# jizongFox/Self-paced-Contrastive-Learning

Measured on AMD Instinct MI355X. Metric: pretrain slices/sec/node (UNet+InfoNCE, 224^2, bs=32/GPU), higher is better.
Workload: dtype bf16; 1 GPU; BASELINE.json configs[1]: self-paced pretrain step, UNet base (max_channel=256) encoder to Conv5 + ProjectionHead(256,256,256) + SelfPacedSupConLoss(soft, partition labels, correct_grad) fwd+bwd + RAdam; slices_per_gpu=32, images_per_gpu_step=64, image=1x224x224, global_batch=32, parallelism=dp1, params=1311056, hipgraph=epocher, capture_steps=3

## Files before the change

### include/spcl_hip.h

```cpp
#ifndef SPCL_HIP_H
#define SPCL_HIP_H
#include <stddef.h>
#include <stdint.h>
#ifdef __cplusplus
extern "C" {
#endif

#define SPCL_F32 0
#define SPCL_BF16 1

#define SPCL_OK 0
#define SPCL_EINVAL (-1)
#define SPCL_ELAUNCH (-2)
#define SPCL_EUNSUPPORTED (-3)

#define SPCL_ABI_VERSION 37
int spcl_abi_version(void);
const char* spcl_last_error(void);

size_t spcl_supcon_workspace_bytes(int n, int d);
int spcl_supcon_forward(const float* z1, const float* z2, const float* labels, const float* mask, int n, int d,
                        float temperature, int sp_mode, float gamma, int correct_grad, float* ws, float* out,
                        void* stream);
int spcl_supcon_backward(const float* labels, const float* mask, int n, int d, float temperature, int sp_mode,
                         float gamma, const float* ws_fwd, float* ws_bwd, const float* out_fwd,
                         const float* grad_out, float* dz1, float* dz2, void* stream);
size_t spcl_supcon_bwd_workspace_bytes(int n, int d);
int spcl_supcon_unit_gradient_block(int n, int d, size_t* offset_floats, int* row_pitch);
int spcl_supcon_forward_heads(int K, const float* z1, const float* z2, size_t z_stride, const float* labels, int n,
                              int d, float temperature, int sp_mode, const float* gammas, int correct_grad, float* ws,
                              size_t ws_stride, float* out, void* stream);
int spcl_supcon_rows_supported(int n, int d);
int spcl_supcon_forward_rows(int K, const float* o1, const float* o2, size_t o_stride, const float* labels, int n, int d,
                             float temperature, int sp_mode, const float* gammas, int correct_grad, float* ws,
                             size_t ws_stride, float* out, void* stream);
int spcl_supcon_backward_heads(int K, const float* labels, int n, int d, float temperature, int sp_mode,
                               const float* gammas, const float* ws_fwd, size_t ws_stride, float* ws_bwd,
                               size_t wsb_stride, const float* out_fwd, const float* grad_out, float* dz1, float* dz2,
                               size_t z_stride, void* stream);
int spcl_supcon_materialize(const float* labels, const float* mask, int n, int d, float temperature, int sp_mode,
                            float gamma, const float* ws_fwd, float* sim_logits, float* sim_exp, float* pos_mask,
                            float* neg_mask, float* sp_mask, void* stream);

size_t spcl_supcon_xpos_workspace_bytes(int n, int d);
int spcl_supcon_xpos_forward(const float* z1, const float* z2, const float* labels, const float* mask, int n, int d,
                             float temperature, float* ws, float* out, void* stream);
int spcl_supcon_xpos_backward(const float* z1, const float* z2, int n, int d, float temperature, const float* ws,
                              const float* grad_out, float* dz1, float* dz2, void* stream);

// ... 188 lines not shown
int spcl_conv3x3_dgrad_bnstats(const void* dy, int dtype, int N, int H, int W, int CinK, int CoutS, const void* w_packed,
                               void* g, const void* y2, const float* scale2, const float* shift2, const float* mean2,
                               float* rows2, void* stream);

int spcl_image_autocorr_rows(int N, int H, int W);
int spcl_image_autocorr(const float* image, int N, int H, int W, float* out, void* stream);
int spcl_conv_dgrad_bnstats_image_supported(int dtype, int N, int H, int W, int CinK, int CoutS);
int spcl_conv3x3_dgrad_bnstats_image(const void* dy, int dtype, int N, int H, int W, int CinK, int CoutS,
                                     const void* w_packed, void* g, const void* y2, const float* scale2,
                                     const float* shift2, const float* mean2, const float* image, float* rows11,
                                     void* stream);
int spcl_conv16_bwd_fused_supported(int dtype, int N, int H, int W, int CinK, int CoutS);
int spcl_conv16_bwd_fused_splits(int N, int H, int W);
int spcl_conv16_bwd_fused(const void* dy, int dtype, int N, int H, int W, const void* w_packed_dgrad, const void* y2,
                          const float* scale2, const float* shift2, const float* mean2, const float* image,
                          float* rows11, float* partial, float* dw_oihw, int Cin, int Cout, float* wg_rows,
                          const float* acorr, int nacorr, float* acorr16, void* stream);
int spcl_conv16_bwd_fused_image_supported(int dtype, int N, int H, int W, int CinK, int CoutS);
int spcl_conv16_bwd_fused_image(const void* dy, int dtype, int N, int H, int W, const void* w_packed_dgrad,
                                const void* w_packed_image, const float* scale2, const float* shift2, const float* mean2,
                                const float* image, float* rows11, float* partial, float* dw_oihw, int Cin, int Cout,
                                float* wg_rows, const float* acorr, int nacorr, float* acorr16, void* stream);
int spcl_conv16_bwd_fused_image_pooled_supported(int dtype, int N, int H, int W, int CinK, int CoutS, int training);
int spcl_conv16_bwd_fused_image_pooled(const void* y, const void* dpool, const float* rows, int nrows, int dtype, int N, int H,
                                       int W, const float* st4, int training, long long* acc, float* dgamma, float* dbeta,
                                       const void* w_packed_dgrad, const void* w_packed_image, const float* scale2,
                                       const float* shift2, const float* mean2, const float* image, float* rows11,
                                       float* partial, float* dw_oihw, int Cin, int Cout, float* wg_rows, const float* acorr,
                                       int nacorr, float* acorr16, void* stream);
int spcl_bnrelu_backward_wgrows_image3(const float* wg_rows, int nwg, const float* acorr, int nacorr, const float* w_oihw,
                                       int N, int H, int W, int C, int CS, const float* mean, const float* invstd,
                                       const float* scale, int training, float* ws, float* dgamma, float* dbeta,
                                       float* dw, void* stream);
size_t spcl_bnrelu_image3_workspace_bytes(int CS);
int spcl_bnrelu_backward_rows_image3(const float* rows11, int nrows, const float* acorr, int nacorr, const float* w_oihw,
                                     int N, int H, int W, int C, int CS, const float* mean, const float* invstd,
                                     const float* scale, int training, float* ws, float* dgamma, float* dbeta, float* dw,
                                     void* stream);

int spcl_conv_dgrad_poolstats_supported(int dtype, int N, int H, int W, int CinK, int CoutS, int H2, int W2);
int spcl_conv3x3_dgrad_poolstats(const void* dy, int dtype, int N, int H, int W, int CinK, int CoutS, const void* w_packed,
                                 void* g, const void* y2, int H2, int W2, const float* scale2, const float* shift2,
                                 const float* mean2, float* rows2, void* stream);
int spcl_bnrelu_pool_backward_rows(const void* y, const void* dpool, const float* rows, int nrows, int dtype, int N, int H,
                                   int W, int C, int CS, const float* mean, const float* invstd, const float* scale,
                                   const float* shift, int training, float* ws, float* dgamma, float* dbeta, void* dy,
                                   void* stream);
int spcl_bnrelu_backward_rows(const void* y, const void* dact, const float* image, const float* rows, int nrows, int dtype,
                              int N, int H, int W, int C, int CS, const float* mean, const float* invstd,
                              const float* scale, const float* shift, int training, float* ws, float* dgamma,
                              float* dbeta, void* dy, float* dw, void* stream);


int spcl_conv1x1_forward(const void* x, int dtype, size_t npix, int C, int CS, int K, const float* w, const float* b,
                         float* out, void* stream);
size_t spcl_conv1x1_bwd_workspace_bytes(int C, int K);
int spcl_conv1x1_backward(const void* x, const float* dout, int dtype, size_t npix, int C, int CS, int K, const float* w,
                          void* dx, float* dw, float* db, float* ws, void* stream);
int spcl_conv1x1_forward_bn(const void* y, int dtype, size_t npix, int C, int CS, int K, const float* scale,
                            const float* shift, const float* w, const float* b, float* out, void* stream);
int spcl_conv1x1_bwd_rows(size_t npix);
int spcl_conv1x1_backward_bn(const void* y, const float* dout, int dtype, size_t npix, int C, int CS, int K,
                             const float* scale, const float* shift, const float* mean, const float* w, void* dact,
                             float* dw, float* db, float* ws, float* rows, void* stream);
int spcl_softmax_forward(const float* logits, size_t npix, int K, float* prob, void* stream);
int spcl_softmax_backward(const float* prob, const float* dprob, size_t npix, int K, float* dlogits, void* stream);
// ... 320 lines not shown
```

### self-paced-contrastive-learning_amd/functional.py

```python
from __future__ import annotations

import collections
import ctypes
import math
import os
import struct
from ctypes import c_double, c_float, c_int

import torch

from . import native as _n

SP_NONE, SP_HARD, SP_SOFT = 0, 1, 2


def take_grad_sink(param, needed: bool = True):
    if not needed or param is None:
        return None
    sink = getattr(param, "_grad_sink", None)
    if sink is None or not getattr(param, "_grad_sink_armed", False):
        return None
    if sink.shape != param.shape or sink.dtype != torch.float32 or not sink.is_contiguous() or sink.device != param.device:
        return None
    param._grad_sink_armed = False
# ... 1150 lines not shown

class DeferredWgrads:

    def __init__(self):
        self.items, self.keep, self.targets = [], [], set()
        self.tails = []

    def add(self, x_store, dy, scale, shift, sink, N, H, W, cin, cin_s, cout, cout_s, in_mode, x2=None, x_up2=False):
        it = _n.WgradItem(x_store.data_ptr(), dy.data_ptr(), scale.data_ptr() if scale is not None else None,
                          shift.data_ptr() if shift is not None else None, sink.data_ptr(), N, H, W, cin, cin_s, cout,
                          cout_s, in_mode, x2.data_ptr() if x2 is not None else None, 1 if x_up2 else 0)
        self.items.append(it)
        self.keep.append((x_store, dy, scale, shift, x2))
        self.targets.add(sink.data_ptr())
        if len(self.items) == _QUEUE_MAX[0]:
            self.flush()

    def capture_tail(self, sink, keep, launch):
        tail = _n.WgradTail()
        _n.call("spcl_wgrad_tail_capture", ctypes.byref(tail))
        try:
            launch()
        finally:
            _n.call("spcl_wgrad_tail_capture", None)
        if tail.kind < 0:
            return False
        self.tails.append(tail)
        self.keep.append(keep)
        self.targets.add(sink.data_ptr())
        if len(self.tails) == _QUEUE_MAX[1]:
            self.flush()
        return True

    def flush(self):
        if not self.items and not self.tails:
            return
        wgrad_batched(self.items, accumulate=False, device=self.keep[0][1].device, tails=self.tails)
        self.items, self.keep, self.tails = [], [], []


_QUEUE_MAX = (min(_n.WGRAD_BATCH_MAX, int(os.environ.get("SPCL_WGRAD_QUEUE_MAX", _n.WGRAD_BATCH_MAX))),
              min(_n.WGRAD_TAILS_MAX, int(os.environ.get("SPCL_WGRAD_QUEUE_MAX", _n.WGRAD_TAILS_MAX))))
_CONV_UP2 = os.environ.get("SPCL_CONV_UP2", "1") != "0"
_UP2_BWD_FUSED = os.environ.get("SPCL_UP2_BWD_FUSED", "1") != "0"
_CONV_SPLIT = os.environ.get("SPCL_CONV_SPLIT", "1") != "0"
_CONV_CAT = os.environ.get("SPCL_CONV_CAT", "1") != "0"
_PACK_AT = os.environ.get("SPCL_PACK_AT", "1") != "0"
_ACC_FILL = os.environ.get("SPCL_ACC_FILL", "1") != "0"
_GAP = os.environ.get("SPCL_GAP", "1") != "0"
_TAILS = os.environ.get("SPCL_WGRAD_TAILS", "1") != "0"


def sink_queue(sink):
    return getattr(sink, "_spcl_queue", None) if sink is not None else None


def wgrad_batched(items, accumulate, device, tails=()):
    arr, ws = None, None
    if items:
        arr = (_n.WgradItem * len(items))(*items)
        nbytes = _n.call("spcl_conv_wgrad_batched_workspace_bytes", arr, len(items))
        if nbytes == 0:
            raise RuntimeError("wgrad_batched: unsupported item (bf16 NHWC, channel counts multiples of 64, in_mode 0/1)")
        ws = torch.empty(nbytes // 4, dtype=torch.float32, device=device)
    tarr = (_n.WgradTail * len(tails))(*tails) if tails else None
    _n.call("spcl_conv3x3_wgrad_batched_tails", arr, len(items), tarr, len(tails), int(bool(accumulate)), _n.ptr(ws),
# ... 124 lines not shown
    dw = _grad_buffer(sinks[0], (C, 1, 3, 3), dev)
    dgamma = _grad_buffer(sinks[1], (C,), dev)
    dbeta = _grad_buffer(sinks[2], (C,), dev)

    def launch():
        _n.call("spcl_bnrelu_backward_image_wgrad", _n.ptr(y), _n.ptr(dact), _n.ptr(image), dt_code, N, H, W, C, cs,
                _n.ptr(st[0]), _n.ptr(st[1]), _n.ptr(st[2]), _n.ptr(st[3]), int(training), _n.ptr(ws), _n.ptr(dgamma),
                _n.ptr(dbeta), _n.ptr(dw), _n.stream())

    queue = sink_queue(sinks[0])
    if queue is not None and _TAILS:
        if queue.capture_tail(sinks[0], (ws, dact), launch):
            dw = None
    else:
        launch()
    return dw, dgamma, dbeta


def _image_wgrad_fusable(cfg, cin, cout_s):
    return cfg.image_input and cin == 1 and cout_s <= 256 and cout_s & (cout_s - 1) == 0


def _dgrad_bnstats(dy, wp_t, y2, st2, dt_code, dtype, N, H, W, cin_k, cout_s):
    if not _n.call("spcl_conv_dgrad_bnstats_supported", dt_code, N, H, W, cin_k, cout_s):
        return None
    dev = dy.device
    nt = _n.call("spcl_conv_stat_rows", dt_code, N, H, W, cin_k, cout_s)
    g = torch.empty(N, H, W, cout_s, dtype=dtype, device=dev)
    rows = torch.empty(nt * 2 * cout_s, dtype=torch.float32, device=dev)
    _n.call("spcl_conv3x3_dgrad_bnstats", _n.ptr(dy), dt_code, N, H, W, cin_k, cout_s, _n.ptr(wp_t), _n.ptr(g),
            _n.ptr(y2), _n.ptr(st2[2]), _n.ptr(st2[3]), _n.ptr(st2[0]), _n.ptr(rows), _n.stream())
    rows.ntiles = nt
    return g, rows


def _bnrelu_bwd_rows(y, dact, image, rows, dt_code, dtype, N, H, W, C, cs, st, training, sinks):
    dev = y.device
    nbytes = _n.call("spcl_bnrelu_image_wgrad_workspace_bytes" if image is not None else
                     "spcl_bnrelu_bwd_workspace_bytes", N, H, W, cs)
    ws = torch.empty(nbytes // 4, dtype=torch.float32, device=dev)
    if image is not None:
        first = _grad_buffer(sinks[0], (C, 1, 3, 3), dev)
        dgamma, dbeta = _grad_buffer(sinks[1], (C,), dev), _grad_buffer(sinks[2], (C,), dev)
        dy, dw = None, first
    else:
        first = torch.empty(N, H, W, cs, dtype=dtype, device=dev)
        dgamma, dbeta = _grad_buffer(sinks[0], (C,), dev), _grad_buffer(sinks[1], (C,), dev)
        dy, dw = first, None
    def launch():
        _n.call("spcl_bnrelu_backward_rows", _n.ptr(y), _n.ptr(dact), _n.ptr(image), _n.ptr(rows), rows.ntiles, dt_code,
                N, H, W, C, cs, _n.ptr(st[0]), _n.ptr(st[1]), _n.ptr(st[2]), _n.ptr(st[3]), int(training), _n.ptr(ws),
                _n.ptr(dgamma), _n.ptr(dbeta), _n.ptr(dy), _n.ptr(dw), _n.stream())

    queue = sink_queue(sinks[0]) if image is not None else None
    if queue is not None and _TAILS:
        if queue.capture_tail(sinks[0], (ws, dact), launch):
            first = None
    else:
        launch()
    return first, dgamma, dbeta


_IMAGE3 = os.environ.get("SPCL_IMAGE3", "1") != "0"


def _image3_supported(cfg, cin, dt_code, N, H, W, cout_s):
# ... 369 lines not shown
                    pooled = (yb, dp_s, lk.rows, stb, acc, dgb.view(cout), dbb.view(cout), cfg.training)
                elif acc is not None:
                    dyb, dgb, dbb = _bnrelu_bwd_rows_acc(yb, None, dp_s, lk.rows, dtc, dtype, N, H, W, cout, cout_s, stb,
                                                         cfg.training, sk[4:6], acc)
                else:
                    dyb, dgb, dbb = _bnrelu_pool_bwd_rows(yb, dp_s, lk.rows, dtc, dtype, N, H, W, cout, cout_s, stb,
                                                          cfg.training, sk[4:6])
        else:
            acc = _take_acc(ctx, "acc_bwd_b") if _ACC_FILL else None
            if acc is not None and lk is not None and lk.rows is ACC_ROWS:
                acc = None
            if acc is not None:
                dyb, dgb, dbb = _bnrelu_bwd_fill(yb, da_s, dp_s, dtc, dtype, N, H, W, cout, cout_s, stb, cfg.training, sk[4:6],
                                                 acc, dact_stride=da_stride, d_up=d_up)
            else:
                dyb, dgb, dbb = _bnrelu_bwd(yb, da_s, dp_s, dtc, dtype, N, H, W, cout, cout_s, stb, cfg.training, sk[4:6],
                                            dact_stride=da_stride, d_up=d_up)
        if lk is not None:
            lk.rows, lk.dx_ptr, lk.holder = None, 0, None
        if la is not None:
            la.rows, la.dx_ptr, la.holder = None, 0, None
        wpa_t, wpb_t = ctx.packed_t
        if wpb_t is None:
            wpb_t = _pack(wb, 1, dtc, dtype)
        image3 = ctx.acorr is not None
        one_pass = (image3 and (_CONV16_FUSED or ya is None) and ctx.needs_input_grad[4] and cout == cout_s
                    and _n.call("spcl_conv16_bwd_fused_supported", dtc, N, H, W, cout_s, cout_s))
        if ya is None and not one_pass:
            raise RuntimeError("image block backward: the first convolution's output was not stored and the one-pass kernel "
                               "that forms it again is not available")
        if pooled is not None and not one_pass:
            raise RuntimeError("image block backward: the gradient behind the max-pool was not materialised and the one-pass "
                               "kernel that forms it is not available")
        if one_pass:
            dwb, rows16 = _conv16_bwd_fused(dyb, wpb_t, ya, sta, xs, dtc, N, H, W, cout, cout, cout_s, sk[3],
                                            acorr=ctx.acorr if _CONV16_WGROWS else None, wp_image=ctx.wpa_fwd, pooled=pooled)
        else:
            dwb = _wgrad(ya, dyb, dtc, N, H, W, cout, cout_s, cout_s, cout, cout_s, 1, sta[2], sta[3], sk[3]) \
                if ctx.needs_input_grad[4] else None
        if one_pass:
            fused = (None, rows16)
        elif image3:
            fused = _dgrad_bnstats_image(dyb, wpb_t, ya, sta, xs, dtc, dtype, N, H, W, cout_s)
        else:
            acc = _take_acc(ctx, "acc_bwd_a")
            if acc is not None:
                fused = (_dgrad_bnstats_acc(dyb, wpb_t, ya, sta, dtc, dtype, N, H, W, cout_s, cout_s, acc), (ACC_ROWS, acc))
            else:
                fused = _dgrad_bnstats(dyb, wpb_t, ya, sta, dtc, dtype, N, H, W, cout_s, cout_s) \
                    if dtype == torch.bfloat16 else None
        if fused is not None:
            daa, rows = fused
        else:
            daa, _ = _conv(dyb, dtc, dtype, N, H, W, cout_s, cout_s, cout_s, wpb_t, 0, None, None, False)
        image_fused = ctx.needs_input_grad[1] and not ctx.needs_input_grad[0] and _image_wgrad_fusable(cfg, cin, cout_s)
        if image3:
            dya = None
            dwa, dga, dba = _bnrelu_bwd_rows_image3(rows, ctx.acorr, wa, N, H, W, cout, cout_s, sta, cfg.training, sk[0:3])
        elif image_fused:
            dya = None
            if fused is not None:
                dwa, dga, dba = _bnrelu_bwd_rows(ya, daa, xs, rows, dtc, dtype, N, H, W, cout, cout_s, sta, cfg.training,
                                                 sk[0:3])
            else:
                dwa, dga, dba = _bnrelu_bwd_image_wgrad(ya, daa, xs, dtc, N, H, W, cout, cout_s, sta, cfg.training,
                                                        sk[0:3])
        else:
            if fused is not None and isinstance(rows, tuple) and rows[0] is ACC_ROWS:
                dya, dga, dba = _bnrelu_bwd_acc(ya, daa, None, None, dtc, dtype, N, H, W, cout, cout_s, sta, cfg.training,
                                                sk[1:3], rows[1])
            elif fused is not None:
                acc = _take_acc(ctx, "acc_rows_a")
                if acc is not None:
                    dya, dga, dba = _bnrelu_bwd_rows_acc(ya, daa, None, rows, dtc, dtype, N, H, W, cout, cout_s, sta,
# ... 2397 lines not shown
```

### self-paced-contrastive-learning_amd/native.py

```python
from __future__ import annotations

import ctypes
import os
from ctypes import c_char_p, c_double, c_float, c_int, c_int64, c_long, c_size_t, c_void_p

import torch

HERE = os.path.dirname(os.path.abspath(__file__))
LIB_PATH = os.path.join(HERE, "lib", "libspcl_hip.so")
SPCL_F32, SPCL_BF16 = 0, 1

_lib = None

_P = c_void_p
_SIGNATURES = {
    "spcl_abi_version": (c_int, []),
    "spcl_last_error": (c_char_p, []),
    "spcl_supcon_workspace_bytes": (c_size_t, [c_int, c_int]),
    "spcl_supcon_forward": (c_int, [_P, _P, _P, _P, c_int, c_int, c_float, c_int, c_float, c_int, _P, _P, _P]),
    "spcl_supcon_backward": (c_int, [_P, _P, c_int, c_int, c_float, c_int, c_float, _P, _P, _P, _P, _P, _P, _P]),
    "spcl_supcon_bwd_workspace_bytes": (c_size_t, [c_int, c_int]),
    "spcl_supcon_unit_gradient_block": (c_int, [c_int, c_int, _P, _P]),
    "spcl_supcon_materialize": (c_int, [_P, _P, c_int, c_int, c_float, c_int, c_float, _P, _P, _P, _P, _P, _P, _P]),
    "spcl_supcon_xpos_workspace_bytes": (c_size_t, [c_int, c_int]),
# ... 80 lines not shown
                                           _P, _P, _P]),
    "spcl_bnrelu_image_wgrad_workspace_bytes": (c_size_t, [c_int, c_int, c_int, c_int]),
    "spcl_bnrelu_backward_image_wgrad": (c_int, [_P, _P, _P, c_int, c_int, c_int, c_int, c_int, c_int, _P, _P, _P, _P,
                                                 c_int, _P, _P, _P, _P, _P]),
    "spcl_accumulate_scalars": (c_int, [c_int, _P, _P, _P, _P]),
    "spcl_stage_bytes": (c_int, [_P, _P, c_size_t, _P]),
    "spcl_conv_dgrad_bnstats_supported": (c_int, [c_int, c_int, c_int, c_int, c_int, c_int]),
    "spcl_conv3x3_dgrad_bnstats": (c_int, [_P, c_int, c_int, c_int, c_int, c_int, c_int, _P, _P, _P, _P, _P, _P, _P, _P]),
    "spcl_conv_dgrad_poolstats_supported": (c_int, [c_int, c_int, c_int, c_int, c_int, c_int, c_int, c_int]),
    "spcl_conv3x3_dgrad_poolstats": (c_int, [_P, c_int, c_int, c_int, c_int, c_int, c_int, _P, _P, _P, c_int, c_int, _P, _P,
                                             _P, _P, _P]),
    "spcl_bnrelu_pool_backward_rows": (c_int, [_P, _P, _P, c_int, c_int, c_int, c_int, c_int, c_int, c_int, _P, _P, _P, _P,
                                               c_int, _P, _P, _P, _P, _P]),
    "spcl_bnrelu_backward_rows": (c_int, [_P, _P, _P, _P, c_int, c_int, c_int, c_int, c_int, c_int, c_int, _P, _P, _P, _P,
                                          c_int, _P, _P, _P, _P, _P, _P]),
    "spcl_image_autocorr_rows": (c_int, [c_int, c_int, c_int]),
    "spcl_image_autocorr": (c_int, [_P, c_int, c_int, c_int, _P, _P]),
    "spcl_conv_dgrad_bnstats_image_supported": (c_int, [c_int, c_int, c_int, c_int, c_int, c_int]),
    "spcl_conv3x3_forward_image_acorr_rows": (c_int, [c_int, c_int, c_int, c_int, c_int, c_int]),
    "spcl_conv3x3_forward_image_acorr": (c_int, [_P, c_int, c_int, c_int, c_int, c_int, c_int, _P, _P, _P, _P, _P]),
    "spcl_block1_recompute_supported": (c_int, [c_int, c_int, c_int, c_int, c_int, c_int]),
    "spcl_block1_kernels_take": (c_int, [c_int, c_int, c_int, c_int, c_int, c_int]),
    "spcl_conv3x3_forward_from_image": (c_int, [_P, _P, c_int, c_int, c_int, c_int, c_int, _P, _P, _P, _P, _P, _P, _P]),
    "spcl_conv16_bwd_fused_image_supported": (c_int, [c_int, c_int, c_int, c_int, c_int, c_int]),
    "spcl_conv16_bwd_fused_image": (c_int, [_P, c_int, c_int, c_int, c_int, _P, _P, _P, _P, _P, _P, _P, _P, _P, c_int, c_int,
                                            _P, _P, c_int, _P, _P]),
    "spcl_conv16_bwd_fused_image_pooled_supported": (c_int, [c_int, c_int, c_int, c_int, c_int, c_int, c_int]),
    "spcl_conv16_bwd_fused_image_pooled": (c_int, [_P, _P, _P, c_int, c_int, c_int, c_int, c_int, _P, c_int, _P, _P, _P, _P, _P,
                                                   _P, _P, _P, _P, _P, _P, _P, c_int, c_int, _P, _P, c_int, _P, _P]),
    "spcl_conv16_bwd_fused_supported": (c_int, [c_int, c_int, c_int, c_int, c_int, c_int]),
    "spcl_conv16_bwd_fused_splits": (c_int, [c_int, c_int, c_int]),
    "spcl_conv16_bwd_fused": (c_int, [_P, c_int, c_int, c_int, c_int, _P, _P, _P, _P, _P, _P, _P, _P, _P, c_int, c_int,
                                      _P, _P, c_int, _P, _P]),
    "spcl_bnrelu_backward_wgrows_image3": (c_int, [_P, c_int, _P, c_int, _P, c_int, c_int, c_int, c_int, c_int, _P, _P, _P,
                                                   c_int, _P, _P, _P, _P, _P]),
    "spcl_conv3x3_dgrad_bnstats_image": (c_int, [_P, c_int, c_int, c_int, c_int, c_int, c_int, _P, _P, _P, _P, _P, _P, _P,
                                                 _P, _P]),
    "spcl_bnrelu_image3_workspace_bytes": (c_size_t, [c_int]),
    "spcl_bnrelu_backward_rows_image3": (c_int, [_P, c_int, _P, c_int, _P, c_int, c_int, c_int, c_int, c_int, _P, _P, _P,
                                                 c_int, _P, _P, _P, _P, _P]),
    "spcl_conv1x1_forward": (c_int, [_P, c_int, c_size_t, c_int, c_int, c_int, _P, _P, _P, _P]),
    "spcl_conv1x1_bwd_workspace_bytes": (c_size_t, [c_int, c_int]),
    "spcl_conv1x1_backward": (c_int, [_P, _P, c_int, c_size_t, c_int, c_int, c_int, _P, _P, _P, _P, _P, _P]),
    "spcl_conv1x1_forward_bn": (c_int, [_P, c_int, c_size_t, c_int, c_int, c_int, _P, _P, _P, _P, _P, _P]),
    "spcl_conv1x1_bwd_rows": (c_int, [c_size_t]),
    "spcl_conv1x1_backward_bn": (c_int, [_P, _P, c_int, c_size_t, c_int, c_int, c_int, _P, _P, _P, _P, _P, _P, _P, _P, _P, _P]),
    "spcl_softmax_forward": (c_int, [_P, c_size_t, c_int, _P, _P]),
    "spcl_softmax_backward": (c_int, [_P, _P, c_size_t, c_int, _P, _P]),
    "spcl_kl_workspace_bytes": (c_size_t, []),
    "spcl_kl_div_forward": (c_int, [_P, _P, c_size_t, c_int, c_float, _P, _P, _P]),
    "spcl_kl_div_backward": (c_int, [_P, _P, c_size_t, c_int, c_float, _P, _P, _P]),
    "spcl_sup_loss_forward": (c_int, [_P, _P, c_int, c_int, c_int, c_float, _P, _P, _P, _P, _P, _P]),
    "spcl_one_hot": (c_int, [_P, c_size_t, c_int, _P, _P]),
    "spcl_argmax_classes": (c_int, [_P, c_size_t, c_int, _P, _P]),
    "spcl_dice_counts": (c_int, [_P, _P, c_int, c_int, c_int, _P, _P, _P]),
    "spcl_surface_workspace_bytes": (c_size_t, [c_int, c_int, c_int, c_int]),
    "spcl_surface_distances": (c_int, [_P, _P, c_int, c_int, c_int, c_int, _P, c_int, c_double, c_double, c_double, _P, _P, _P,
                                       _P, _P, c_size_t, _P]),
    "spcl_surface_3d_workspace_bytes": (c_size_t, [c_int, c_int, c_int, c_int, c_int]),
    "spcl_surface_distances_3d": (c_int, [_P, _P, c_int, c_int, c_int, c_int, c_int, _P, c_int, c_double, c_double, c_double,
                                          c_double, _P, _P, _P, _P, _P, c_size_t, _P]),
    "spcl_largest_component_workspace_bytes": (c_size_t, [c_int, c_int, c_int, c_int, c_int]),
    "spcl_largest_component": (c_int, [_P, c_int, c_int, c_int, c_int, c_int, _P, c_int, _P, _P, _P, _P, c_size_t, _P]),
    "spcl_tta_merge_workspace_bytes": (c_size_t, [c_int, c_int, c_int]),
    "spcl_tta_merge": (c_int, [_P, _P, c_int, c_int, c_int, c_int, c_int, c_float, _P, _P, _P, _P, _P, c_size_t, _P]),
    "spcl_embed_monitor_workspace_bytes": (c_size_t, [c_int, c_int, c_int]),
# ... 148 lines not shown
class WgradItem(ctypes.Structure):
    _fields_ = [("x", c_void_p), ("dy", c_void_p), ("in_scale", c_void_p), ("in_shift", c_void_p),
                ("dw_oihw", c_void_p), ("N", c_int), ("H", c_int), ("W", c_int), ("Cin", c_int), ("CinS", c_int),
                ("Cout", c_int), ("CoutS", c_int), ("in_mode", c_int), ("x2", c_void_p), ("x_up2", c_int)]


class PackItem(ctypes.Structure):
    _fields_ = [("w_oihw", c_void_p), ("fwd", c_void_p), ("dgrad", c_void_p), ("Cin", c_int), ("Cout", c_int),
                ("H", c_int), ("W", c_int)]


BN_EVAL_MAX = 32


class BnEvalItem(ctypes.Structure):
    _fields_ = [("gamma", c_void_p), ("beta", c_void_p), ("running_mean", c_void_p), ("running_var", c_void_p),
                ("st", c_void_p), ("C", c_int), ("CS", c_int), ("eps", c_float)]


class BnAcc(ctypes.Structure):
    _fields_ = [("acc", c_void_p), ("gamma", c_void_p), ("beta", c_void_p), ("running_mean", c_void_p),
                ("running_var", c_void_p), ("num_batches_tracked", c_void_p), ("st", c_void_p), ("momentum", c_float),
                ("eps", c_float), ("count", c_float), ("C", c_int), ("CS", c_int)]


PACK_MULTI_MAX = 24


class WgradTail(ctypes.Structure):
    _fields_ = [("partial", c_void_p), ("dw", c_void_p), ("kind", c_int), ("nsplit", c_int), ("nblk_ci", c_int),
                ("nblk_co", c_int), ("CIB", c_int), ("COB", c_int), ("Cin", c_int), ("Cout", c_int)]


ABI_VERSION = 37
WGRAD_BATCH_MAX = 16
WGRAD_TAILS_MAX = 16
_NO_STATUS = ("spcl_abi_version", "spcl_block1_recompute_supported", "spcl_block1_kernels_take", "spcl_conv16_bwd_fused_image_supported", "spcl_conv3x3_forward_image_acorr_rows", "spcl_image_autocorr_rows", "spcl_conv_dgrad_bnstats_image_supported", "spcl_conv16_bwd_fused_supported", "spcl_conv16_bwd_fused_splits", "spcl_conv_num_tiles", "spcl_conv_stat_rows", "spcl_conv_set_gemm", "spcl_conv_set_f32_split", "spcl_conv_get_f32_split", "spcl_supcon_unit_gradient_block", "spcl_conv_cat_supported", "spcl_conv_up2_supported", "spcl_conv_split_supported", "spcl_conv_split_bnstats_supported", "spcl_conv1x1_bwd_rows", "spcl_profile_count", "spcl_conv_dgrad_bnstats_supported", "spcl_conv_dgrad_poolstats_supported",
              "spcl_conv_wgrad_batched_supported", "spcl_conv_bn_acc_supported", "spcl_conv_dgrad_bnstats_acc_supported",
              "spcl_conv_dgrad_poolstats_acc_supported", "spcl_supcon_rows_supported", "spcl_bnrelu_gap_supported",
              "spcl_conv_dgrad_poolmax_supported", "spcl_conv_dgrad_poolmax_acc_supported",
              "spcl_conv16_bwd_fused_image_pooled_supported")


class NativeLibraryError(RuntimeError):
    pass


def lib():
    global _lib
    if _lib is None:
        if not os.path.exists(LIB_PATH):
            raise NativeLibraryError(
                f"{LIB_PATH} is missing: build it with `python self-paced-contrastive-learning_amd/build.py` "
                "(there is no CPU / eager fallback for the hot path)")
        L = ctypes.CDLL(LIB_PATH)
        L.spcl_abi_version.restype, L.spcl_abi_version.argtypes = c_int, []
        have = L.spcl_abi_version()
        if have != ABI_VERSION:
            raise NativeLibraryError(
                f"{LIB_PATH} has C-ABI version {have}, this binding was written for {ABI_VERSION} (include/spcl_hip.h "
                "SPCL_ABI_VERSION): a stale build -- rebuild with `python self-paced-contrastive-learning_amd/build.py`")
        for name, (res, args) in _SIGNATURES.items():
            fn = getattr(L, name, None)
            if fn is None:
                continue
            fn.restype, fn.argtypes = res, args
        _lib = L
    return _lib


def call(name: str, *args):
    L = lib()
    fn = getattr(L, name, None)
    if fn is None:
# ... 35 lines not shown
```

Before: 32390 slices/s.

## Fuse 32-channel conv3x3 backward dgrad, BN stats and wgrad into one pass

Adds a HIP kernel for the 32->32 channel 3x3 conv in the second encoder block that computes the data gradient, the BN/ReLU backward statistics rows, and the weight-gradient partials in one persistent pass. Each dy halo tile is loaded into LDS once and reused for both MFMA dgrad and transposed-read wgrad, with double-buffered prefetch of the next tile. The path is enabled by default in the block backward when shapes fit (bf16, H%7, W%14). This replaces separate wgrad and dgrad+bnstats launches, cutting repeated reads of dy and y2. The cost is a large specialised kernel, per-workgroup partials that need a reduce tail, and possible occupancy limits from heavy register use.

```diff
diff --git a/include/spcl_hip.h b/include/spcl_hip.h
--- a/include/spcl_hip.h
+++ b/include/spcl_hip.h
@@ -14,7 +14,7 @@
 #define SPCL_ELAUNCH (-2)
 #define SPCL_EUNSUPPORTED (-3)
 
-#define SPCL_ABI_VERSION 37
+#define SPCL_ABI_VERSION 38
 int spcl_abi_version(void);
 const char* spcl_last_error(void);
 
@@ -269,6 +269,12 @@
                                        int N, int H, int W, int C, int CS, const float* mean, const float* invstd,
                                        const float* scale, int training, float* ws, float* dgamma, float* dbeta,
                                        float* dw, void* stream);
+int spcl_conv3x3_bwd_fused_supported(int dtype, int N, int H, int W, int CinK, int CoutS, int training);
+int spcl_conv3x3_bwd_fused_workgroups(int N, int H, int W, int max_workgroups);
+int spcl_conv3x3_bwd_fused(const void* dy, int dtype, int N, int H, int W, int CinK, int CoutS, const void* w_packed_dgrad,
+                           const void* y2, const float* scale2, const float* shift2, const float* mean2, void* g,
+                           float* rows2, float* partial, float* dw_oihw, int Cin, int Cout, spcl_wgrad_tail* tail,
+                           int max_workgroups, void* stream);
 size_t spcl_bnrelu_image3_workspace_bytes(int CS);
 int spcl_bnrelu_backward_rows_image3(const float* rows11, int nrows, const float* acorr, int nacorr, const float* w_oihw,
                                      int N, int H, int W, int C, int CS, const float* mean, const float* invstd,
diff --git a/self-paced-contrastive-learning_amd/csrc/conv32_bwd.hip b/self-paced-contrastive-learning_amd/csrc/conv32_bwd.hip
--- /dev/null
+++ b/self-paced-contrastive-learning_amd/csrc/conv32_bwd.hip
@@ -0,0 +1,336 @@
+#include "conv_common.hpp"
+
+namespace spcl {
+
+struct Bwd32Args {
+  const unsigned char* dy;
+  const u32x4* wp;
+  const unsigned char* y2;
+  const float* scale2;
+  const float* shift2;
+  const float* mean2;
+  unsigned char* g;
+  float* rows2;
+  float* partial;
+  int N, H, W, tilesX, tilesY, ntiles, nwg;
+};
+
+typedef __attribute__((ext_vector_type(2))) uint32_t u32x2;
+
+constexpr int B32_TH = 7, B32_TW = 14, B32_RP = 18, B32_PS = 96, B32_HROWS = 10;
+constexpr int B32_DY = 0, B32_DY_BYTES = B32_HROWS * B32_RP * B32_PS;
+constexpr int B32_XPS = 96, B32_XROW = 16 * B32_XPS;
+constexpr int B32_XT = B32_DY + 2 * B32_DY_BYTES, B32_XT_BYTES = 8 * B32_XROW;
+constexpr int B32_RED = B32_XT + B32_XT_BYTES;
+constexpr int B32_TRASH = B32_RED + 4096;
+constexpr int B32_LDS = B32_TRASH + 64;
+constexpr int B32_MAX_WG = 512;
+
+__device__ __forceinline__ bf16x8 b32_tr_frag(unsigned addr, int hi_off) {
+  const s16x4 lo = __builtin_amdgcn_ds_read_tr16_b64_v4i16((s16x4 __attribute__((address_space(3)))*)(uintptr_t)addr);
+  const s16x4 hi = __builtin_amdgcn_ds_read_tr16_b64_v4i16((s16x4 __attribute__((address_space(3)))*)(uintptr_t)(addr + hi_off));
+  return __builtin_shufflevector(lo, hi, 0, 1, 2, 3, 4, 5, 6, 7);
+}
+
+__global__ __launch_bounds__(256) __attribute__((amdgpu_waves_per_eu(2))) void conv32_bwd_kernel(Bwd32Args a) {
+  constexpr int TH = B32_TH, TW = B32_TW, RP = B32_RP, PS = B32_PS, XPS = B32_XPS, XROW = B32_XROW;
+  constexpr int OOB = (int)0x80000000u;
+  extern __shared__ __attribute__((aligned(16))) unsigned char lds[];
+  const unsigned lds_base = (unsigned)(uintptr_t)(unsigned char __attribute__((address_space(3)))*)lds;
+  const int t0 = threadIdx.x;
+  const int wave = __builtin_amdgcn_readfirstlane(t0 >> 6);
+  const int nt = wave & 1, half = wave >> 1;
+  const int wg = blockIdx.x;
+  const int tbeg = (int)((long)wg * a.ntiles / a.nwg), tend = (int)((long)(wg + 1) * a.ntiles / a.nwg);
+  const int tpi = a.tilesX * a.tilesY;
+
+  u32x4 wfr[9];
+#pragma unroll
+  for (int s = 0; s < 9; ++s) wfr[s] = a.wp[(size_t)(s * 2 + nt) * 64 + (t0 & 63)];
+  const int cb = nt * 16 + 4 * ((t0 & 63) >> 4);
+  const f32x4 sc2 = *(const f32x4*)(a.scale2 + cb), sh2 = *(const f32x4*)(a.shift2 + cb), mu2 = *(const f32x4*)(a.mean2 + cb);
+
+  for (int i = t0; i < (2 * B32_DY_BYTES + B32_XT_BYTES) / 16; i += 256) *(u32x4*)(lds + i * 16) = (u32x4){0u, 0u, 0u, 0u};
+
+  const int u0 = half ? (nt ? 5 : 0) : (nt ? 14 : 10);
+  f32x4 wacc[5][2];
+#pragma unroll
+  for (int j = 0; j < 5; ++j) wacc[j][0] = wacc[j][1] = (f32x4){0.f, 0.f, 0.f, 0.f};
+  unsigned ax, ad[5];
+  {
+    const int lane = t0 & 63, r16 = lane & 15, gq = lane >> 4;
+    ax = lds_base + B32_XT + (gq >> 1) * XROW + (4 * (gq & 1) + (r16 >> 2)) * XPS + (r16 & 3) * 8;
+#pragma unroll
+    for (int j = 0; j < 5; ++j) {
+      const int u = min(u0 + j, 17), tap = u >> 1, nj = u & 1, ky = tap / 3, kx = tap - 3 * ky;
+      ad[j] = lds_base + B32_DY + (((gq >> 1) + 2 - ky) * RP + 4 * (gq & 1) + (r16 >> 2) + 2 - kx) * PS + (r16 & 3) * 8 + nj * 32;
+    }
+  }
+
+  auto rsrc = [](const void* p) { return __builtin_amdgcn_make_buffer_rsrc((void*)p, 0, 0x7fffffff, 0x00020000); };
+  u32x4 v[3];
+  u32x2 ypre[4];
+  auto issue_halo = [&](const int n, const int y0, const int x0, const bool live) {
+    int t = t0;
+    asm volatile("" : "+v"(t));
+    const int ch = t & 3, hx = (t >> 2) & 15, hy0 = t >> 6;
+    const __amdgpu_buffer_rsrc_t rs = rsrc(a.dy + (((long)n * a.H + (y0 - 1)) * a.W + (x0 - 1)) * 64);
+    const int gx = x0 - 1 + hx;
+    const bool colok = gx >= 0 && gx < a.W;
+    const int voff = (hy0 * a.W + hx) * 64 + ch * 16;
+#pragma unroll
+    for (int k = 0; k < 3; ++k) {
+      const int hy = hy0 + 4 * k, gy = y0 - 1 + hy;
+      const bool ok = live && colok && hy < TH + 2 && gy >= 0 && gy < a.H;
+      v[k] = __builtin_bit_cast(u32x4, __builtin_amdgcn_raw_buffer_load_b128(rs, ok ? voff : OOB, 4 * k * a.W * 64, 0));
+    }
+  };
+  auto issue_y2 = [&](const int n, const int y0, const int x0, const bool live) {
+    int t = t0;
+    asm volatile("" : "+v"(t));
+    const int r16 = t & 15, gq = (t & 63) >> 4;
+    const __amdgpu_buffer_rsrc_t rs = rsrc(a.y2 + (((long)n * a.H + y0) * a.W + x0) * 64);
+    const int voff = r16 * 64 + nt * 32 + gq * 8;
+#pragma unroll
+    for (int j = 0; j < 4; ++j) {
+      const int i = 4 * half + j;
+      ypre[j] = __builtin_bit_cast(u32x2, __builtin_amdgcn_raw_buffer_load_b64(rs, (live && r16 < TW && i < TH) ? voff : OOB, i * a.W * 64, 0));
+    }
+  };
+
+  auto drop_store = [&]() {
+    __builtin_amdgcn_raw_buffer_store_b64((u32x2){0u, 0u}, rsrc(a.g), OOB, 0, 0);
+  };
+  int cn = tbeg / tpi, cy0, cx0;
+  {
+    const int rem = tbeg - cn * tpi, ty = rem / a.tilesX;
+    cy0 = ty * TH;
+    cx0 = (rem - ty * a.tilesX) * TW;
+  }
+  issue_halo(cn, cy0, cx0, tbeg < tend);
+  drop_store(); drop_store(); drop_store(); drop_store();
+  issue_y2(cn, cy0, cx0, tbeg < tend);
+  drop_store();
+  int hoff = 0;
+  {
+    u32x4 wx = wfr[0];
+#pragma unroll
+    for (int s = 1; s < 9; ++s) wx ^= wfr[s];
+    *(u32x4*)(lds + B32_TRASH) = wx;
+    *(f32x4*)(lds + B32_TRASH + 16) = sc2 + sh2 + mu2;
+  }
+  __syncthreads();
+
+#pragma unroll 1
+  for (int tile = tbeg; tile < tend; ++tile) {
+    const int n = cn, y0 = cy0, x0 = cx0;
+    cx0 += TW;
+    if (cx0 == a.W) {
+      cx0 = 0;
+      cy0 += TH;
+      if (cy0 == a.H) {
+        cy0 = 0;
+        cn += 1;
+      }
+    }
+    int t = t0;
+    asm volatile("" : "+v"(t));
+    const int lane = t & 63, r16 = lane & 15, gq = lane >> 4;
+    const bool more = tile + 1 < tend;
+    {
+      const int ch = t & 3, hx = (t >> 2) & 15, hy0 = t >> 6;
+      unsigned char* const lp = lds + B32_DY + hoff + (hy0 * RP + hx) * PS + ch * 16;
+      *(u32x4*)lp = v[0];
+      *(u32x4*)(lp + 4 * RP * PS) = v[1];
+      *(u32x4*)(lds + B32_DY + hoff + (min(hy0 + 8, 9) * RP + hx) * PS + ch * 16) = v[2];
+    }
+    issue_halo(cn, cy0, cx0, more);
+    __builtin_amdgcn_sched_barrier(0);
+    __syncthreads();
+
+    f32x4 acc[4];
+    {
+      const unsigned char* const ab = lds + B32_DY + hoff + ((4 * half) * RP + r16) * PS + gq * 16;
+#pragma unroll
+      for (int j = 0; j < 4; ++j) acc[j] = (f32x4){0.f, 0.f, 0.f, 0.f};
+#pragma unroll
+      for (int s = 0; s < 9; ++s) {
+        const int off = ((s / 3) * RP + (s % 3)) * PS;
+#pragma unroll
+        for (int j = 0; j < 3; ++j) acc[j] = mfma_chunk<bf16_t>(wfr[s], *(const u32x4*)(ab + j * RP * PS + off), acc[j]);
+      }
+      if (half == 0) {
+#pragma unroll
+        for (int s = 0; s < 9; ++s) {
+          const int off = ((s / 3) * RP + (s % 3)) * PS;
+          acc[3] = mfma_chunk<bf16_t>(wfr[s], *(const u32x4*)(ab + 3 * RP * PS + off), acc[3]);
+        }
+      }
+    }
+    __builtin_amdgcn_sched_barrier(0);
+
+    const bool act = r16 < TW;
+    float dz[4][4], dd[4][4];
+    u32x2 gpk[4];
+#pragma unroll
+    for (int j = 0; j < 4; ++j) {
+      const bool rowok = j < 3 || half == 0;
+      const int i = 4 * half + j;
+      const u32x2 yr = ypre[j];
+      const float yv[4] = {__uint_as_float(yr.x << 16), __uint_as_float(yr.x & 0xffff0000u),
+                           __uint_as_float(yr.y << 16), __uint_as_float(yr.y & 0xffff0000u)};
+      const f32x2 glo = {acc[j][0], acc[j][1]}, ghi = {acc[j][2], acc[j][3]};
+      const uint32_t g0 = __builtin_bit_cast(uint32_t, __builtin_convertvector(glo, bf16x2v));
+      const uint32_t g1 = __builtin_bit_cast(uint32_t, __builtin_convertvector(ghi, bf16x2v));
+      const float gv[4] = {__uint_as_float(g0 << 16), __uint_as_float(g0 & 0xffff0000u),
+                           __uint_as_float(g1 << 16), __uint_as_float(g1 & 0xffff0000u)};
+      gpk[j] = (u32x2){g0, g1};
+      float z[4];
+#pragma unroll
+      for (int r = 0; r < 4; ++r) {
+        z[r] = fmaf(sc2[r], yv[r], sh2[r]);
+        dz[j][r] = (act && rowok && z[r] > 0.f) ? gv[r] : 0.f;
+        dd[j][r] = (act && rowok) ? yv[r] - mu2[r] : 0.f;
+      }
+      const f32x2 zlo = {z[0], z[1]}, zhi = {z[2], z[3]};
+      u32x2 xw;
+      xw.x = relu_bf16x2(__builtin_bit_cast(uint32_t, __builtin_convertvector(zlo, bf16x2v)));
+      xw.y = relu_bf16x2(__builtin_bit_cast(uint32_t, __builtin_convertvector(zhi, bf16x2v)));
+      if (!(act && rowok)) xw = (u32x2){0u, 0u};
+      *(u32x2*)(lds + B32_XT + i * XROW + r16 * XPS + nt * 32 + gq * 8) = xw;
+    }
+    {
+      const __amdgpu_buffer_rsrc_t rs = rsrc(a.g + (((size_t)n * a.H + y0) * a.W + x0) * 64);
+      const int voff = r16 * 64 + nt * 32 + gq * 8;
+#pragma unroll
+      for (int j = 0; j < 4; ++j)
+        __builtin_amdgcn_raw_buffer_store_b64(gpk[j], rs, (act && (j < 3 || half == 0)) ? voff : OOB, (4 * half + j) * a.W * 64, 0);
+    }
+    issue_y2(cn, cy0, cx0, more);
+    f32x4* const red = (f32x4*)(lds + B32_RED + (nt * 64 + lane) * 32);
+    if (half == 0) {
+      f32x4 ssum = {0.f, 0.f, 0.f, 0.f}, ssq = {0.f, 0.f, 0.f, 0.f};
+#pragma unroll
+      for (int j = 0; j < 4; ++j)
+#pragma unroll
+        for (int r = 0; r < 4; ++r) {
+          ssum[r] += dz[j][r];
+          ssq[r] = fmaf(dz[j][r], dd[j][r], ssq[r]);
+        }
+      red[0] = ssum;
+      red[1] = ssq;
+    }
+    __builtin_amdgcn_sched_barrier(0);
+    __syncthreads();
+    f32x4 o = {0.f, 0.f, 0.f, 0.f};
+    if (half != 0) {
+      f32x4 ssum = red[0], ssq = red[1];
+#pragma unroll
+      for (int j = 0; j < 3; ++j)
+#pragma unroll
+        for (int r = 0; r < 4; ++r) {
+          ssum[r] += dz[j][r];
+          ssq[r] = fmaf(dz[j][r], dd[j][r], ssq[r]);
+        }
+#pragma unroll
+      for (int r = 0; r < 4; ++r) {
+        const float s1 = row16_sum(ssum[r]), s2 = row16_sum(ssq[r]);
+        o[r] = r16 == 0 ? s1 : s2;
+      }
+    }
+    __builtin_amdgcn_raw_buffer_store_b128(__builtin_bit_cast(u32x4, o), rsrc(a.rows2 + (size_t)tile * 64),
+                                           (half != 0 && r16 < 2) ? (r16 * 32 + nt * 16 + 4 * gq) * 4 : OOB, 0, 0);
+    __builtin_amdgcn_sched_barrier(0);
+
+    {
+      bf16x8 fa[2][2], fb[2][5];
+      auto load_ks = [&](const int ks, const int b) {
+        fa[b][0] = b32_tr_frag(ax + ks * 2 * XROW, 8 * XPS);
+        fa[b][1] = b32_tr_frag(ax + ks * 2 * XROW + 32, 8 * XPS);
+#pragma unroll
+        for (int j = 0; j < 5; ++j) fb[b][j] = b32_tr_frag(ad[j] + hoff + ks * 2 * RP * PS, 8 * PS);
+      };
+      load_ks(0, 0);
+#pragma unroll
+      for (int ks = 0; ks < 4; ++ks) {
+        if (ks + 1 < 4) load_ks(ks + 1, (ks + 1) & 1);
+#pragma unroll
+        for (int j = 0; j < 5; ++j) {
+          wacc[j][0] = __builtin_amdgcn_mfma_f32_16x16x32_bf16(fa[ks & 1][0], fb[ks & 1][j], wacc[j][0], 0, 0, 0);
+          wacc[j][1] = __builtin_amdgcn_mfma_f32_16x16x32_bf16(fa[ks & 1][1], fb[ks & 1][j], wacc[j][1], 0, 0, 0);
+        }
+      }
+    }
+    __builtin_amdgcn_sched_barrier(0);
+    hoff ^= B32_DY_BYTES;
+  }
+
+  float* const out = a.partial + (size_t)wg * (9 * 32 * 32);
+  const int r16 = t0 & 15, gq = (t0 & 63) >> 4;
+#pragma unroll
+  for (int j = 0; j < 5; ++j) {
+    if (j == 4 && half == 0) continue;
+    const int u = u0 + j, tap = u >> 1, nj = u & 1;
+#pragma unroll
+    for (int mi = 0; mi < 2; ++mi)
+#pragma unroll
+      for (int r = 0; r < 4; ++r) out[(tap * 32 + mi * 16 + 4 * gq + r) * 32 + nj * 16 + r16] = wacc[j][mi][r];
+  }
+}
+
+static int bwd32_workgroups(int N, int H, int W, int max_workgroups) {
+  if (N <= 0 || H < B32_TH || W < B32_TW || H % B32_TH != 0 || W % B32_TW != 0) return 0;
+  const long tiles = (long)N * (H / B32_TH) * (W / B32_TW);
+  long nwg = 2 * 256;
+  if (nwg > B32_MAX_WG) nwg = B32_MAX_WG;
+  if (nwg > tiles) nwg = tiles;
+  if (max_workgroups > 0 && nwg > max_workgroups) nwg = max_workgroups;
+  return (int)nwg;
+}
+
+}
+
+using namespace spcl;
+
+extern "C" int spcl_conv3x3_bwd_fused_supported(int dtype, int N, int H, int W, int CinK, int CoutS, int training) {
+  if (dtype != SPCL_BF16 || !training || CinK != 32 || CoutS != 32) return 0;
+  if (N <= 0 || H < B32_TH || W < B32_TW || H % B32_TH != 0 || W % B32_TW != 0) return 0;
+  if ((double)H * W * 64.0 >= 2147483648.0) return 0;
+  if (!spcl_conv_dgrad_bnstats_supported(dtype, N, H, W, CinK, CoutS)) return 0;
+  return spcl_conv_stat_rows(dtype, N, H, W, CinK, CoutS) == N * (H / B32_TH) * (W / B32_TW) ? 1 : 0;
+}
+
+extern "C" int spcl_conv3x3_bwd_fused_workgroups(int N, int H, int W, int max_workgroups) {
+  return bwd32_workgroups(N, H, W, max_workgroups);
+}
+
+extern "C" int spcl_conv3x3_bwd_fused(const void* dy, int dtype, int N, int H, int W, int CinK, int CoutS,
+                                      const void* w_packed_dgrad, const void* y2, const float* scale2, const float* shift2,
+                                      const float* mean2, void* g, float* rows2, float* partial, float* dw_oihw, int Cin,
+                                      int Cout, spcl_wgrad_tail* tail, int max_workgroups, void* stream) {
+  SPCL_CHECK_ARG(dy && w_packed_dgrad && y2 && scale2 && shift2 && mean2 && g && rows2 && partial && (dw_oihw || tail),
+                 "conv3x3_bwd_fused: null pointer");
+  SPCL_CHECK_ARG(Cin > 0 && Cin <= 32 && Cout > 0 && Cout <= 32 && max_workgroups >= 0, "conv3x3_bwd_fused: channel counts");
+  if (!spcl_conv3x3_bwd_fused_supported(dtype, N, H, W, CinK, CoutS, 1)) {
+    set_error("conv3x3_bwd_fused: unsupported configuration (bf16, 32 -> 32 channels, H %% 7 == 0, W %% 14 == 0)");
+    return SPCL_EUNSUPPORTED;
+  }
+  hipStream_t st = (hipStream_t)stream;
+  Bwd32Args a;
+  a.dy = (const unsigned char*)dy; a.wp = (const u32x4*)w_packed_dgrad; a.y2 = (const unsigned char*)y2;
+  a.scale2 = scale2; a.shift2 = shift2; a.mean2 = mean2; a.g = (unsigned char*)g; a.rows2 = rows2; a.partial = partial;
+  a.N = N; a.H = H; a.W = W; a.tilesX = W / B32_TW; a.tilesY = H / B32_TH; a.ntiles = N * a.tilesX * a.tilesY;
+  a.nwg = bwd32_workgroups(N, H, W, max_workgroups);
+  const double px = (double)N * H * W;
+  prof_cost(px * (32 * 2.0 + 32 * 2.0) + 9.0 * Cin * Cout * 4.0 + px * (32 + 2.0 * 32) * 2.0 + 9.0 * 32 * 32 * 2.0,
+            2.0 * px * 9.0 * Cin * Cout + 2.0 * px * 9.0 * 32 * 32);
+  SPCL_LAUNCH(conv32_bwd_kernel, dim3(a.nwg), dim3(256), B32_LDS, st, a);
+  if (tail != nullptr) {
+    tail->partial = partial; tail->dw = dw_oihw; tail->kind = 0; tail->nsplit = a.nwg; tail->nblk_ci = 1;
+    tail->nblk_co = 1; tail->CIB = 32; tail->COB = 32; tail->Cin = Cin; tail->Cout = Cout;
+  } else {
+    launch_wgrad_reduce(partial, a.nwg, 1, 1, 32, 32, Cin, Cout, dw_oihw, st);
+  }
+  SPCL_LAUNCH_CHECK("conv3x3_bwd_fused");
+  return SPCL_OK;
+}
diff --git a/self-paced-contrastive-learning_amd/functional.py b/self-paced-contrastive-learning_amd/functional.py
--- a/self-paced-contrastive-learning_amd/functional.py
+++ b/self-paced-contrastive-learning_amd/functional.py
@@ -1206,6 +1206,13 @@
             self.flush()
         return True
 
+    def add_tail(self, tail, sink, keep):
+        self.tails.append(tail)
+        self.keep.append(keep)
+        self.targets.add(sink.data_ptr())
+        if len(self.tails) == _QUEUE_MAX[1]:
+            self.flush()
+
     def flush(self):
         if not self.items and not self.tails:
             return
@@ -1396,6 +1403,32 @@
             _n.ptr(y2), _n.ptr(st2[2]), _n.ptr(st2[3]), _n.ptr(st2[0]), _n.ptr(rows), _n.stream())
     rows.ntiles = nt
     return g, rows
+
+
+_BLOCK2B_ONE_PASS = os.environ.get("SPCL_BLOCK2B_ONE_PASS", "1") != "0"
+
+
+def _conv32_bwd_fused(dy, wp_t, y2, st2, dt_code, dtype, N, H, W, c, cs, sink=None, max_workgroups=0):
+    dev = dy.device
+    nwg = _n.call("spcl_conv3x3_bwd_fused_workgroups", N, H, W, max_workgroups)
+    nt = _n.call("spcl_conv_stat_rows", dt_code, N, H, W, cs, cs)
+    g = torch.empty(N, H, W, cs, dtype=dtype, device=dev)
+    rows = torch.empty(nt * 2 * cs, dtype=torch.float32, device=dev)
+    rows.ntiles = nt
+    ws = torch.empty(nwg * 9 * 32 * 32, dtype=torch.float32, device=dev)
+    dw = _grad_buffer(sink, (c, c, 3, 3), dev)
+    queue = sink_queue(sink)
+    tail = None
+    if queue is not None and _TAILS:
+        tail = _n.WgradTail()
+        tail.kind = -1
+    _n.call("spcl_conv3x3_bwd_fused", _n.ptr(dy), dt_code, N, H, W, cs, cs, _n.ptr(wp_t), _n.ptr(y2), _n.ptr(st2[2]),
+            _n.ptr(st2[3]), _n.ptr(st2[0]), _n.ptr(g), _n.ptr(rows), _n.ptr(ws), _n.ptr(dw), c, c,
+            ctypes.byref(tail) if tail is not None else None, max_workgroups, _n.stream())
+    if tail is not None:
+        queue.add_tail(tail, sink, (ws, dy, y2, st2))
+        dw = None
+    return dw, (g, rows)
 
 
 def _bnrelu_bwd_rows(y, dact, image, rows, dt_code, dtype, N, H, W, C, cs, st, training, sinks):
@@ -1831,14 +1864,21 @@
         if pooled is not None and not one_pass:
             raise RuntimeError("image block backward: the gradient behind the max-pool was not materialised and the one-pass "
                                "kernel that forms it is not available")
+        one_pass32 = bool(not one_pass and not image3 and _BLOCK2B_ONE_PASS and ctx.needs_input_grad[4] and ya is not None
+                          and dtype == torch.bfloat16 and getattr(ctx, "acc_bwd_a", None) is None
+                          and _n.call("spcl_conv3x3_bwd_fused_supported", dtc, N, H, W, cout_s, cout_s, int(cfg.training)))
         if one_pass:
             dwb, rows16 = _conv16_bwd_fused(dyb, wpb_t, ya, sta, xs, dtc, N, H, W, cout, cout, cout_s, sk[3],
                                             acorr=ctx.acorr if _CONV16_WGROWS else None, wp_image=ctx.wpa_fwd, pooled=pooled)
+        elif one_pass32:
+            dwb, fused32 = _conv32_bwd_fused(dyb, wpb_t, ya, sta, dtc, dtype, N, H, W, cout, cout_s, sk[3])
         else:
             dwb = _wgrad(ya, dyb, dtc, N, H, W, cout, cout_s, cout_s, cout, cout_s, 1, sta[2], sta[3], sk[3]) \
                 if ctx.needs_input_grad[4] else None
         if one_pass:
             fused = (None, rows16)
+        elif one_pass32:
+            fused = fused32
         elif image3:
             fused = _dgrad_bnstats_image(dyb, wpb_t, ya, sta, xs, dtc, dtype, N, H, W, cout_s)
         else:
diff --git a/self-paced-contrastive-learning_amd/native.py b/self-paced-contrastive-learning_amd/native.py
--- a/self-paced-contrastive-learning_amd/native.py
+++ b/self-paced-contrastive-learning_amd/native.py
@@ -136,6 +136,10 @@
     "spcl_conv16_bwd_fused_splits": (c_int, [c_int, c_int, c_int]),
     "spcl_conv16_bwd_fused": (c_int, [_P, c_int, c_int, c_int, c_int, _P, _P, _P, _P, _P, _P, _P, _P, _P, c_int, c_int,
                                       _P, _P, c_int, _P, _P]),
+    "spcl_conv3x3_bwd_fused_supported": (c_int, [c_int, c_int, c_int, c_int, c_int, c_int, c_int]),
+    "spcl_conv3x3_bwd_fused_workgroups": (c_int, [c_int, c_int, c_int, c_int]),
+    "spcl_conv3x3_bwd_fused": (c_int, [_P, c_int, c_int, c_int, c_int, c_int, c_int, _P, _P, _P, _P, _P, _P, _P, _P, _P, c_int,
+                                       c_int, _P, c_int, _P]),
     "spcl_bnrelu_backward_wgrows_image3": (c_int, [_P, c_int, _P, c_int, _P, c_int, c_int, c_int, c_int, c_int, _P, _P, _P,
                                                    c_int, _P, _P, _P, _P, _P]),
     "spcl_conv3x3_dgrad_bnstats_image": (c_int, [_P, c_int, c_int, c_int, c_int, c_int, c_int, _P, _P, _P, _P, _P, _P, _P,
@@ -350,14 +354,15 @@
                 ("nblk_co", c_int), ("CIB", c_int), ("COB", c_int), ("Cin", c_int), ("Cout", c_int)]
 
 
-ABI_VERSION = 37
+ABI_VERSION = 38
 WGRAD_BATCH_MAX = 16
 WGRAD_TAILS_MAX = 16
 _NO_STATUS = ("spcl_abi_version", "spcl_block1_recompute_supported", "spcl_block1_kernels_take", "spcl_conv16_bwd_fused_image_supported", "spcl_conv3x3_forward_image_acorr_rows", "spcl_image_autocorr_rows", "spcl_conv_dgrad_bnstats_image_supported", "spcl_conv16_bwd_fused_supported", "spcl_conv16_bwd_fused_splits", "spcl_conv_num_tiles", "spcl_conv_stat_rows", "spcl_conv_set_gemm", "spcl_conv_set_f32_split", "spcl_conv_get_f32_split", "spcl_supcon_unit_gradient_block", "spcl_conv_cat_supported", "spcl_conv_up2_supported", "spcl_conv_split_supported", "spcl_conv_split_bnstats_supported", "spcl_conv1x1_bwd_rows", "spcl_profile_count", "spcl_conv_dgrad_bnstats_supported", "spcl_conv_dgrad_poolstats_supported",
               "spcl_conv_wgrad_batched_supported", "spcl_conv_bn_acc_supported", "spcl_conv_dgrad_bnstats_acc_supported",
               "spcl_conv_dgrad_poolstats_acc_supported", "spcl_supcon_rows_supported", "spcl_bnrelu_gap_supported",
               "spcl_conv_dgrad_poolmax_supported", "spcl_conv_dgrad_poolmax_acc_supported",
-              "spcl_conv16_bwd_fused_image_pooled_supported")
+              "spcl_conv16_bwd_fused_image_pooled_supported", "spcl_conv3x3_bwd_fused_supported",
+              "spcl_conv3x3_bwd_fused_workgroups")
 
 
 class NativeLibraryError(RuntimeError):
```

After: 32680 slices/s, median of 6. About the same (+0.9%).
